# JeffOwOSun/ntm-tracker

Hardware: AMD Instinct MI355X
Metric: frames/sec (whole node) VGG16+NTM(128x20) seq_len=20 (higher is better)
Workload: dtype f32

## Files before the change

### ntm-tracker_amd/csrc/conv_bf16p.hip

```cpp
#include "conv_tiles.h"
#include "conv_stem.h"

#ifndef BF16P_ABL
#define BF16P_ABL 0
#endif

namespace {

typedef __bf16 pbf16x8 __attribute__((ext_vector_type(8)));
typedef __bf16 pbf16x4 __attribute__((ext_vector_type(4)));


struct Bf16pArgs {
    const __bf16* in; const __bf16* wq; const float* bias; void* out;
    int frames, H, W, Cin, Cout;
    int bxN, byN;
    int NQ, NS;
    int nCB;
    const float* stem_in = nullptr; const float* stem_w = nullptr; const float* stem_b = nullptr;
};

typedef int pv4i __attribute__((ext_vector_type(4)));
__device__ __forceinline__ void p_dma16(pv4i rs, unsigned lds_addr, int voff, int soff) {
    unsigned keep;
    asm volatile("s_mov_b32 %0, m0\n\ts_mov_b32 m0, %1\n\ts_nop 0\n\tbuffer_load_dwordx4 %2, %3, %4 offen lds\n\ts_mov_b32 m0, %0"
                 : "=&s"(keep) : "s"(lds_addr), "v"(voff), "s"(rs), "s"(soff) : "memory");
}
__device__ __forceinline__ pv4i p_rsrc(const void* base, unsigned bytes) {
    const unsigned long long p = (unsigned long long)base;
    return pv4i{(int)(unsigned)p, (int)(unsigned)(p >> 32), (int)bytes, 0x00020000};
}

__device__ __forceinline__ pbf16x8 p_as_bf16x8(const f32x4& v) {
    union { f32x4 f; pbf16x8 b; } u;
    u.f = v;
    return u.b;
}

typedef _Float16 ph16x8 __attribute__((ext_vector_type(8)));
typedef _Float16 ph16x4 __attribute__((ext_vector_type(4)));
typedef _Float16 ph16x2 __attribute__((ext_vector_type(2)));
__device__ __forceinline__ ph16x8 p_as_f16x8(const f32x4& v) {
    union { f32x4 f; ph16x8 h; } u;
    u.f = v;
    return u.h;
}
__device__ __forceinline__ void s3_split4(const f32x4& v, ph16x4& hi, ph16x4& lo) {
    const auto h01 = __builtin_amdgcn_cvt_pkrtz(v[0], v[1]), h23 = __builtin_amdgcn_cvt_pkrtz(v[2], v[3]);
    hi = ph16x4{(_Float16)h01[0], (_Float16)h01[1], (_Float16)h23[0], (_Float16)h23[1]};
#pragma unroll
    for (int e = 0; e < 4; ++e) lo[e] = (_Float16)(v[e] - (float)hi[e]);
}
constexpr float S3_MAX = 131008.f;

template <int PIECES>
__device__ __forceinline__ int p_sw(int idx) { return PIECES == 4 ? ((idx >> 2) & 3) : ((idx >> 3) & 1); }

template <int BN, int KC>
__global__ void bf16p_pack_kernel(const float* __restrict__ w, __bf16* __restrict__ wq, int Cin, int Cout) {
// ... 24 lines not shown
    for (int o = 32; o > 0; o >>= 1) m = fmaxf(m, __shfl_xor(m, o));
    if ((threadIdx.x & 63) == 0) atomicMax(tail + 1, __float_as_uint(m));
}
__global__ void split3_scale_kernel(unsigned* __restrict__ tail) {
    const float m = __uint_as_float(tail[1]);
    int e = 0;
    if (m > 0.f) frexpf(m, &e);
    int k = 14 - e;
    k = k > 100 ? 100 : (k < -100 ? -100 : k);
    reinterpret_cast<float*>(tail)[0] = ldexpf(1.f, -k);
    reinterpret_cast<float*>(tail)[2] = ldexpf(1.f, k);
}
template <int BN>
__global__ void split3_pack_kernel(const float* __restrict__ w, _Float16* __restrict__ wq, int Cin, int Cout) {
    const size_t total = (size_t)18 * Cin * Cout;
    const float wscale = reinterpret_cast<const float*>(wq + total)[2];
    const int NC = Cin / 16;
    for (size_t idx = (size_t)blockIdx.x * blockDim.x + threadIdx.x; idx < total; idx += (size_t)gridDim.x * blockDim.x) {
        const int e = idx & 7;
        size_t r = idx >> 3;
        const int slot = (int)(r & 3); r >>= 2;
        const int n = (int)(r % BN); r /= BN;
        const int tap = (int)(r % 9); r /= 9;
        const int chunk = (int)(r % NC);
        const int cb = (int)(r / NC);
        const int piece = slot ^ p_sw<4>(n);
        const int c = chunk * 16 + (piece & 1) * 8 + e;
        const float v = w[((size_t)tap * Cin + c) * Cout + (size_t)cb * BN + n] * wscale;
        const _Float16 hi = (_Float16)v;
        wq[idx] = (piece & 2) ? (_Float16)(v - (float)hi) : hi;
    }
}

template <int BN, int TW, int TH, int NSUB, int KC, bool POOL, bool OUTF32, int NW = 8, bool X3 = false, bool INF32 = false, bool STEM = false>
__global__ __launch_bounds__(64 * NW) __attribute__((amdgpu_waves_per_eu(2, 2))) void conv3x3_relu_bf16p_kernel(Bf16pArgs a) {
    static_assert(!INF32 || (X3 && NW == 4), "fp32 input: split form on four waves (the eight-wave form has no registers for the staging)");
    static_assert(!STEM || (X3 && NW == 4 && !INF32 && (TW & (TW - 1)) == 0 && TW % 2 == 0), "fused stem: split form on four waves, sub-blocks");
    constexpr int PNT = 2 * NW;
    constexpr bool ROWS = (TW & (TW - 1)) != 0;
    static_assert(!X3 || KC == 32, "split form: 16 real channels = one 32-channel chunk");
    static_assert(!ROWS || (!POOL && NSUB == 1 && (TW - 1 + 32 * PNT - 1) / TW + 1 <= TH - 1 && NW == 8), "runs of rows: no row pairs; TH = the patch's image rows");
    static_assert(NW == 8 || (NW == 4 && BN == 64), "four-wave workgroups take 64 columns");
    constexpr int PW = ROWS ? 32 : TW + 2, PH = TH + 2, SPX = PW * PH, NPX = NSUB * SPX;
    static_assert(!ROWS || TW + 2 <= 32, "runs of rows: the patch row pitch is 32");
    constexpr int PIXB = KC * 2, PIECES = KC / 8, PPP = 1024 / PIXB;
    constexpr int NPA = (NPX + PPP - 1) / PPP;
    constexpr int ABYTES = STEM ? NPX * PIXB : NPA * 1024;
    constexpr int STAPS = KC == 16 ? 9 : 3, SPC = 9 / STAPS;
    constexpr int SBYTES = STAPS * BN * PIXB, NPB = SBYTES / 1024;
    constexpr int NPAW = (NPA + NW - 1) / NW;
    constexpr int TM = BN == 128 ? 4 : 2;
    constexpr int TPS = (TW * TH) / 32;
    constexpr int K16 = KC / 16;
    static_assert(ROWS || NSUB * TW * TH == 32 * PNT, "512 (256) output pixels per workgroup");
    constexpr int TRB = POOL ? 0 : NW * TM * 32 * 144;
    constexpr int LDSB = (2 * ABYTES + 2 * SBYTES) > TRB ? (2 * ABYTES + 2 * SBYTES) : TRB;
    constexpr int FPW = TW + 4, FPN = STEM ? NSUB * (TH + 4) * FPW * 3 : 4;
    constexpr int STEMB = STEM ? (FPN + 4 * 27 * 16 + 64) * 4 : 0;
    static_assert(LDSB + STEMB + 1024 <= ((NW == 8 || (STEM && NSUB > 1)) ? 160 : 80) * 1024, "LDS");
    __shared__ __attribute__((aligned(16))) float s_fp[FPN];
    __shared__ __attribute__((aligned(16))) float s_w1[STEM ? 4 * 27 * 16 : 4];
    __shared__ __attribute__((aligned(16))) float s_b1[STEM ? 64 : 4];
    __shared__ __attribute__((aligned(1024))) unsigned char s_mem[LDSB];
    __shared__ int s_sbf[NSUB], s_sby[NSUB], s_sbx[NSUB];
    __shared__ __attribute__((aligned(16))) float s_bias[BN + 4];

    const int tid = threadIdx.x, lane = tid & 63;
    const int wave = __builtin_amdgcn_readfirstlane(tid >> 6);
    int cb, sp;
    conv_tile_wg(blockIdx.x, a.nCB, cb, sp);
    if (sp >= a.NS) return;
    const int H = a.H, W = a.W, Cin = a.Cin, Cout = a.Cout;
    const int rP0 = sp * (32 * PNT), rg0 = ROWS ? rP0 / TW : 0, rf0 = ROWS ? rg0 / H : 0, ry0 = ROWS ? rg0 - rf0 * H : 0;
    if (tid < BN) s_bias[tid] = a.bias[cb * BN + tid];
    if (X3 && tid == BN) s_bias[BN] = *reinterpret_cast<const float*>(a.wq + (size_t)9 * a.Cin * a.Cout);
    if constexpr (!ROWS) conv_tile_subblocks<NSUB>(s_sbf, s_sby, s_sbx, tid, sp, a.NQ, a.bxN, a.byN, TH, TW, 0, 0);
    if constexpr (STEM) {
        for (int e = tid; e < 4 * 27 * 16; e += 64 * NW) {
            const int k = (e >> 4) % 27;
            s_w1[e] = a.stem_w[((e / (27 * 16)) * 16 + (e & 15)) * 32 + k];
        }
        if (tid < 64) s_b1[tid] = a.stem_b[tid];
    }
    __syncthreads();
    if constexpr (STEM) {
        for (int e = tid; e < FPN; e += 64 * NW) {
            int q, fy, fx, c, y, x;
            stem_fp_elem(e, TW, TH, q, fy, fx, c);
            const bool in = stem_fp_src(fy, fx, s_sby[q], s_sbx[q], H, W, y, x) && s_sbf[q] >= 0;
            s_fp[e] = in ? a.stem_in[(((size_t)s_sbf[q] * H + y) * W + x) * 3 + c] : 0.f;
        }
        __syncthreads();
    }

    auto a_sw = [](int p) { return ROWS ? ((((p & 31) + 28 * (p >> 5)) >> 2) & 3) : p_sw<PIECES>(p); };
    const int f0 = ROWS ? rf0 : ((sp * NSUB) / a.bxN) / a.byN;
    const size_t in_left = (size_t)(a.frames - f0) * H * W * Cin * sizeof(__bf16);
    const unsigned in_bytes = (unsigned)(in_left < 0x7ffffff0ull ? in_left : 0x7ffffff0ull);
    const __bf16* pin = a.in + (size_t)f0 * H * W * Cin;
    unsigned aoff[NPAW];
#pragma unroll
    for (int i = 0; i < NPAW; ++i) {
        const int pa = wave + NW * i;
        const int lp = pa * PPP + lane / PIECES, slot = lane % PIECES;
        aoff[i] = 0x80000000u;
        if (pa < NPA && lp < NPX) {
            const int q = lp / SPX, rem = lp - q * SPX;
            const int py = rem / PW, px = rem - py * PW;
            int fq, y;
            const int x = (ROWS ? 0 : s_sbx[q]) - 1 + px;
            if constexpr (ROWS) {
                const int U = ry0 + py, df = U / (H + 1);
                fq = rf0 + df; y = U - df * (H + 1) - 1;
                if (fq >= a.frames) fq = -1;
            } else {
                fq = s_sbf[q]; y = s_sby[q] - 1 + py;
            }
            if (fq >= 0 && y >= 0 && y < H && x >= 0 && x < W)
                aoff[i] = (unsigned)(((((size_t)(fq - f0) * H + y) * W + x) * Cin + (slot ^ a_sw(lp)) * 8) * sizeof(__bf16));
        }
    }
    constexpr int NIT = INF32 ? (NPX * 4 + 64 * NW - 1) / (64 * NW) : 1;
    constexpr int NITS = (NIT + SPC - 1) / SPC;
    unsigned foff[NIT];
    int fdst[NIT];
    if constexpr (INF32) {
#pragma unroll
        for (int i = 0; i < NIT; ++i) {
            const int it = tid + 64 * NW * i, lp = it >> 2, qd = it & 3;
            foff[i] = 0x80000000u; fdst[i] = -1;
            if (lp < NPX) {
                fdst[i] = lp * PIXB + (((qd >> 1) ^ a_sw(lp)) << 4) + (qd & 1) * 8;
                const int q = lp / SPX, rem = lp - q * SPX;
                const int py = rem / PW, px = rem - py * PW;
                const int fq = s_sbf[q];
                const int y = s_sby[q] - 1 + py, x = s_sbx[q] - 1 + px;
                if (fq >= 0 && y >= 0 && y < H && x >= 0 && x < W)
                    foff[i] = (unsigned)(((((size_t)(fq - f0) * H + y) * W + x) * Cin) * sizeof(__bf16) + qd * 16);
            }
        }
    }
    auto f32_rsrc = [&](int chunk) {
        return __builtin_amdgcn_make_buffer_rsrc(const_cast<__bf16*>(pin + (size_t)chunk * KC), 0, (int)(in_bytes - (unsigned)chunk * PIXB), 0x00020000);
    };
    auto f32_put = [&](const f32x4& v, int dst) {
        ph16x4 h, l;
        f32x4 c;
#pragma unroll
        for (int e = 0; e < 4; ++e) c[e] = __builtin_amdgcn_fmed3f(v[e], -S3_MAX, S3_MAX);
        s3_split4(c, h, l);
        *reinterpret_cast<ph16x4*>(s_mem + dst) = h;
        *reinterpret_cast<ph16x4*>(s_mem + (dst ^ 32)) = l;
    };
    constexpr int STILES = (NPX + 15) / 16;
// ... 67 lines not shown
    auto dma_weights = [&](int stage, int buf) {
#pragma unroll
        for (int i = 0; i < (NPB + NW - 1) / NW; ++i) {
            const int pb = wave + NW * i;
            if (pb < NPB) p_dma16(wrs, lds0 + 2 * ABYTES + buf * SBYTES + pb * 1024, lane * 16, stage * SBYTES + pb * 1024);
        }
    };

    const int wm = BN == 128 ? (wave >> 1) : wave, wn = BN == 128 ? (wave & 1) : 0;
    const int mcol = lane & 31, kh = lane >> 5;
    int pix0[TM];
    int opix[TM];
    auto locate = [&](int t, int m, int& pc, int& op) {
        if constexpr (ROWS) {
            const int P = rP0 + t * 32 + m;
            const int g = P / TW, x = P - g * TW, f = g / H, y = g - f * H;
            const bool real = f < a.frames;
            pc = real ? ((f - rf0) * (H + 1) + y + 1 - ry0) * PW + x + 1 : PW + 1;
            op = real ? P : -1;
        } else {
            int q, y, x;
            if constexpr (TPS == 0) {
                q = 2 * t + (m >> 4); y = (m >> 2) & 3; x = m & 3;
            } else {
                constexpr int RPT = 32 / TW;
                const int tl = t % TPS, j = m / TW;
                q = t / TPS;
                y = 2 * ((tl >> 1) * RPT + j) + (tl & 1);
                x = m % TW;
                if constexpr (TW == 16) x = (x + 12 * j) & 15;
                if constexpr (TW == 8) x ^= ((0x9 >> j) & 1) << 2;
            }
            pc = q * SPX + (y + 1) * PW + (x + 1);
            const int fq = s_sbf[q];
            const int Y = s_sby[q] + y, X = s_sbx[q] + x;
            if constexpr (POOL) op = fq < 0 ? -1 : ((fq * (H >> 1) + (Y >> 1)) * (W >> 1) + (X >> 1));
            else op = fq < 0 ? -1 : ((fq * H + Y) * W + X);
        }
    };
#pragma unroll
    for (int tm = 0; tm < TM; ++tm) locate(wm * TM + tm, mcol, pix0[tm], opix[tm]);
    int xa[9][TM];
#pragma unroll
    for (int tap = 0; tap < 9; ++tap)
#pragma unroll
        for (int tm = 0; tm < TM; ++tm) {
            const int p = pix0[tm] + (tap / 3 - 1) * PW + (tap % 3 - 1);
            xa[tap][tm] = p * PIXB + ((kh ^ a_sw(p)) << 4);
        }
    f32x16 acc[TM][2];
#pragma unroll
    for (int tm = 0; tm < TM; ++tm)
#pragma unroll
        for (int nt = 0; nt < 2; ++nt)
#pragma unroll
            for (int r = 0; r < 16; ++r) acc[tm][nt][r] = 0.f;
    const int wa0 = 2 * ABYTES + (wn * 64 + mcol) * PIXB + ((kh ^ p_sw<PIECES>(mcol)) << 4);

    if constexpr (INF32) {
        const __amdgpu_buffer_rsrc_t rs = f32_rsrc(0);
        f32x4 v[NIT];
#pragma unroll
        for (int i = 0; i < NIT; ++i) v[i] = __builtin_bit_cast(f32x4, __builtin_amdgcn_raw_buffer_load_b128(rs, (int)foff[i], 0, 0));
#pragma unroll
        for (int i = 0; i < NIT; ++i)
            if (fdst[i] >= 0) f32_put(v[i], fdst[i]);
    } else if constexpr (!STEM) {
        dma_patch(0, 0, 0, NPAW);
    }
    dma_weights(0, 0);
    if constexpr (STEM) {
#pragma unroll
        for (int i = 0; i < SNIT; ++i) {
            stem_load(0, i, 0);
#pragma unroll
            for (int s = 0; s < 7; ++s) stem_mfma(0, s);
            stem_put(i, 0, 0);
        }
    }
    asm volatile("s_waitcnt vmcnt(0)" ::: "memory");
    __syncthreads();

    auto stage_body = [&](int chunk, auto part_c) {
        constexpr int part = decltype(part_c)::value;
        const int s = SPC * chunk + part;
        const int abuf = chunk & 1, bbuf = s & 1;
        constexpr int NDW = (NPB + NW - 1) / NW;
        constexpr int NDP = (INF32 || STEM) ? 0 : (NPAW + SPC - 1) / SPC;
        const bool more_w = !(BF16P_ABL & 1) && s + 1 < NSTG, more_p = !(BF16P_ABL & 1) && chunk + 1 < NC;
        auto dma_slot = [&](auto kc) {
            constexpr int k = decltype(kc)::value;
            if constexpr (k < NDW) { if (more_w) dma_weights1(s + 1, bbuf ^ 1, k); }
            else if constexpr (k < NDW + NDP && part * NDP + (k - NDW) < NPAW) {
                if (more_p) dma_patch1(chunk + 1, abuf ^ 1, ntk_ic<part * NDP + (k - NDW)>{});
            }
        };
        constexpr int SPER = (7 * SNITS + 8) / 9;
        auto stem_slot = [&](auto kc) {
            if constexpr (STEM) {
                constexpr int k = decltype(kc)::value;
                if (more_p) {
#pragma unroll
                    for (int u = k * SPER; u < (k + 1) * SPER && u < 7 * SNITS; ++u) {
                        if (part * SNITS + u / 7 >= SNIT) continue;
                        stem_mfma(u / 7, u % 7);
                        if (u % 7 == 6) stem_put(part * SNITS + u / 7, u / 7, abuf ^ 1);
                    }
                }
            }
        };
        if constexpr (STEM) {
            if (more_p) {
#pragma unroll
                for (int j = 0; j < SNITS; ++j)
                    if (part * SNITS + j < SNIT) stem_load(chunk + 1, part * SNITS + j, j);
            }
        }
        const int wa = wa0 + bbuf * SBYTES;
        f32x4 fst[NITS];
        if constexpr (INF32) {
            const __amdgpu_buffer_rsrc_t rs = f32_rsrc(more_p ? chunk + 1 : chunk);
#pragma unroll
            for (int j = 0; j < NITS; ++j)
                if (part * NITS + j < NIT) fst[j] = __builtin_bit_cast(f32x4, __builtin_amdgcn_raw_buffer_load_b128(rs, (int)foff[part * NITS + j], 0, 0));
        }
        if constexpr (X3) {
            f32x4 wh[2][2], wl[2], xh[TM], xl[TM];
// ... 30 lines not shown
                __builtin_amdgcn_sched_barrier(0);
                if constexpr (!(BF16P_ABL & 4)) ld_x(dc, I1{}, xl);
                __builtin_amdgcn_sched_barrier(0);
                mm(wl, xh);
                dma_slot(ntk_ic<3 * dxi + 1>{});
                stem_slot(ntk_ic<3 * dxi + 1>{});
                __builtin_amdgcn_sched_barrier(0);
                if constexpr (dxi + 1 < STAPS && !(BF16P_ABL & 4)) {
                    ld_w(ntk_ic<dxi + 1>{}, I0{}, wh[(dxi + 1) & 1]);
                    ld_x(ntk_ic<dxi + 1>{}, I0{}, xh);
                }
                __builtin_amdgcn_sched_barrier(0);
                mm(wh[dxi & 1], xl);
                dma_slot(ntk_ic<3 * dxi + 2>{});
                stem_slot(ntk_ic<3 * dxi + 2>{});
                __builtin_amdgcn_sched_barrier(0);
            };
            ld_w(I0{}, I0{}, wh[0]);
            ld_x(I0{}, I0{}, xh);
            if constexpr ((BF16P_ABL & 4) != 0) {
#pragma unroll
                for (int nt = 0; nt < 2; ++nt) { wh[1][nt] = wh[0][nt]; wl[nt] = wh[0][nt]; }
#pragma unroll
                for (int tm = 0; tm < TM; ++tm) xl[tm] = xh[tm];
            }
            ntk_static_for<0, STAPS>(tapstep);
            if constexpr (INF32) {
                if (more_p) {
#pragma unroll
                    for (int j = 0; j < NITS; ++j)
                        if (part * NITS + j < NIT && fdst[part * NITS + j] >= 0) f32_put(fst[j], (abuf ^ 1) * ABYTES + fdst[part * NITS + j]);
                }
            }
            if (!(BF16P_ABL & 2)) {
                asm volatile("s_waitcnt vmcnt(0)" ::: "memory");
                __syncthreads();
            }
            return;
        }
        constexpr int NSTEP = STAPS * K16;
        f32x4 wf[2][2], xf[2][TM];
        auto load_frags = [&](auto stc, f32x4 (&wfs)[2], f32x4 (&xfs)[TM]) {
            constexpr int st = decltype(stc)::value, dxi = st / K16, k16 = st % K16;
            constexpr int tap = part * STAPS + dxi;
#pragma unroll
            for (int nt = 0; nt < 2; ++nt)
                wfs[nt] = *reinterpret_cast<const f32x4*>(s_mem + ((wa ^ (k16 << 5)) + (dxi * BN + nt * 32) * PIXB));
#pragma unroll
            for (int tm = 0; tm < TM; ++tm) xfs[tm] = *reinterpret_cast<const f32x4*>(s_mem + (xa[tap][tm] ^ (k16 << 5)));
        };
        auto step = [&](auto stc) {
            constexpr int st = decltype(stc)::value;
            if constexpr (st + 1 < NSTEP && !(BF16P_ABL & 4)) load_frags(ntk_ic<st + 1>{}, wf[(st + 1) & 1], xf[(st + 1) & 1]);
            __builtin_amdgcn_sched_barrier(0);
            if constexpr ((BF16P_ABL & 8) != 0) return;
#pragma unroll
            for (int tm = 0; tm < TM; ++tm)
#pragma unroll
                for (int nt = 0; nt < 2; ++nt)
                    acc[tm][nt] = __builtin_amdgcn_mfma_f32_32x32x16_bf16(p_as_bf16x8(wf[(BF16P_ABL & 4) ? 0 : (st & 1)][nt]),
                                                                          p_as_bf16x8(xf[(BF16P_ABL & 4) ? 0 : (st & 1)][tm]), acc[tm][nt], 0, 0, 0);
            constexpr int PER = (NDW + NDP + NSTEP - 1) / NSTEP;
            dma_slot(ntk_ic<st * PER>{});
            if constexpr (PER > 1) dma_slot(ntk_ic<st * PER + 1>{});
            static_assert(PER <= 2, "DMAs per step");
            __builtin_amdgcn_sched_barrier(0);
        };
        if (!(BF16P_ABL & 4) || s == 0) load_frags(ntk_ic<0>{}, wf[0], xf[0]);
        ntk_static_for<0, NSTEP>(step);
        if (!(BF16P_ABL & 2)) {
            asm volatile("s_waitcnt vmcnt(0)" ::: "memory");
            __syncthreads();
        }
    };
    for (int chunk = 0; chunk < NC; ++chunk) {
        stage_body(chunk, ntk_ic<0>{});
        if constexpr (SPC > 1) {
            stage_body(chunk, ntk_ic<1>{});
            stage_body(chunk, ntk_ic<2>{});
        }
        const int flip = (chunk & 1) ? -ABYTES : ABYTES;
#pragma unroll
        for (int tap = 0; tap < 9; ++tap)
#pragma unroll
            for (int tm = 0; tm < TM; ++tm) xa[tap][tm] += flip;
    }

    if constexpr ((BF16P_ABL & 16) != 0) {
        float sacc = 0.f;
#pragma unroll
        for (int tm = 0; tm < TM; ++tm)
#pragma unroll
            for (int nt = 0; nt < 2; ++nt)
#pragma unroll
                for (int r = 0; r < 16; ++r) sacc += acc[tm][nt][r];
        if (sacc == 12345.f) reinterpret_cast<float*>(a.out)[tid] = sacc;
        return;
    }
    const int nbase = cb * BN + wn * 64 + 4 * kh;
    const float oscale = X3 ? s_bias[BN] : 1.f;
    if constexpr (POOL) {
#pragma unroll
        for (int nt = 0; nt < 2; ++nt)
#pragma unroll
            for (int g = 0; g < 4; ++g) {
                const int n = nbase + nt * 32 + 8 * g;
                const f32x4 bv = *reinterpret_cast<const f32x4*>(s_bias + n - cb * BN);
#pragma unroll
                for (int tm = 0; tm < TM; tm += 2) {
                    f32x4 v;
#pragma unroll
                    for (int e = 0; e < 4; ++e) {
                        const float m2 = fmaxf(acc[tm][nt][4 * g + e], acc[tm + 1][nt][4 * g + e]);
                        const float m4 = fmaxf(m2, ntk_dpp<0xB1>(m2));
                        if constexpr (X3 && !OUTF32) v[e] = __builtin_amdgcn_fmed3f(m4 * oscale + bv[e], 0.f, S3_MAX);
                        else v[e] = fmaxf((X3 ? m4 * oscale : m4) + bv[e], 0.f);
                    }
                    if (opix[tm] >= 0 && (mcol & 1) == 0) {
                        if constexpr (OUTF32) *reinterpret_cast<f32x4*>(reinterpret_cast<float*>(a.out) + (size_t)opix[tm] * Cout + n) = v;
                        else if constexpr (X3) {
                            ph16x4 oh, ol;
                            s3_split4(v, oh, ol);
                            _Float16* op = reinterpret_cast<_Float16*>(a.out) + (size_t)opix[tm] * (2 * Cout) + (n >> 4) * 32 + (n & 15);
                            *reinterpret_cast<ph16x4*>(op) = oh;
                            *reinterpret_cast<ph16x4*>(op + 16) = ol;
                        } else {
                            pbf16x4 o;
#pragma unroll
                            for (int e = 0; e < 4; ++e) o[e] = (__bf16)v[e];
                            *reinterpret_cast<pbf16x4*>(reinterpret_cast<__bf16*>(a.out) + (size_t)opix[tm] * Cout + n) = o;
                        }
                    }
                }
            }
    } else {
        constexpr int RB = 144;
        constexpr int WREG = TM * 32 * RB;
        static_assert(NW * WREG <= LDSB, "the transpose image fits");
        unsigned char* tr = s_mem + wave * WREG;
        constexpr bool WIDE = OUTF32 || X3;
        constexpr int NPASS = WIDE ? 2 : 1;
#pragma unroll
        for (int ps = 0; ps < NPASS; ++ps) {
#pragma unroll
            for (int nt = 0; nt < 2; ++nt) {
                if (WIDE && nt != ps) continue;
#pragma unroll
                for (int g = 0; g < 4; ++g) {
                    const f32x4 bv = *reinterpret_cast<const f32x4*>(s_bias + nbase - cb * BN + nt * 32 + 8 * g);
#pragma unroll
                    for (int tm = 0; tm < TM; ++tm) {
                        f32x4 v;
#pragma unroll
                        for (int e = 0; e < 4; ++e) {
                            if constexpr (X3 && !OUTF32) v[e] = __builtin_amdgcn_fmed3f(acc[tm][nt][4 * g + e] * oscale + bv[e], 0.f, S3_MAX);
                            else v[e] = fmaxf((X3 ? acc[tm][nt][4 * g + e] * oscale : acc[tm][nt][4 * g + e]) + bv[e], 0.f);
                        }
                        unsigned char* row = tr + (tm * 32 + mcol) * RB;
                        if constexpr (OUTF32) *reinterpret_cast<f32x4*>(row + (8 * g + 4 * kh) * 4) = v;
                        else if constexpr (X3) {
                            ph16x4 oh, ol;
                            s3_split4(v, oh, ol);
                            unsigned char* pr = row + (g >> 1) * 64 + ((g & 1) * 8 + 4 * kh) * 2;
                            *reinterpret_cast<ph16x4*>(pr) = oh;
                            *reinterpret_cast<ph16x4*>(pr + 32) = ol;
                        } else {
                            pbf16x4 o;
#pragma unroll
                            for (int e = 0; e < 4; ++e) o[e] = (__bf16)v[e];
                            *reinterpret_cast<pbf16x4*>(row + (nt * 32 + 8 * g + 4 * kh) * 2) = o;
                        }
                    }
                }
            }
#pragma unroll
            for (int j = 0; j < TM * 4; ++j) {
                const int tmr = j >> 2, mr = 8 * (j & 3) + (lane >> 3), piece = lane & 7;
                const f32x4 v = *reinterpret_cast<const f32x4*>(tr + (tmr * 32 + mr) * RB + piece * 16);
                const int opx = __builtin_amdgcn_ds_bpermute(mr << 2, opix[tmr]);
                if ((BF16P_ABL & 32) ? (opx >= 0 && v[0] == 12345.f) : (opx >= 0)) {
                    const size_t op = (size_t)opx * Cout + cb * BN + wn * 64;
                    if constexpr (OUTF32) *reinterpret_cast<f32x4*>(reinterpret_cast<float*>(a.out) + op + ps * 32 + piece * 4) = v;
                    else if constexpr (X3) *reinterpret_cast<f32x4*>(reinterpret_cast<__bf16*>(a.out) + 2 * (op + ps * 32) + piece * 8) = v;
                    else *reinterpret_cast<f32x4*>(reinterpret_cast<__bf16*>(a.out) + op + piece * 8) = v;
                }
            }
        }
    }
}

template <int BN, int KC, int NW, bool X3 = false, bool INF32 = false, bool STEM = false>
int bf16p_launch(const Bf16pArgs& a0, int H, int W, int pool, int out_f32, hipStream_t st) {
    Bf16pArgs a = a0;
    if constexpr (X3 && !INF32) {
        if (W == 28) {
            if (pool || NW != 8 || H < 20) return NTK_ERR_UNSUPPORTED;
            a.bxN = 1; a.byN = 1;
            const long long NQ = (long long)a.frames * H * W, NS = (NQ + 511) / 512;
            a.NQ = 0; a.NS = (int)NS; a.nCB = a.Cout / BN;
            const unsigned grid = (unsigned)conv_tile_grid(NS, a.nCB);
            if constexpr (NW == 8) {
                if (out_f32) conv3x3_relu_bf16p_kernel<BN, 28, 21, 1, 32, false, true, 8, true><<<grid, 512, 0, st>>>(a);
                else conv3x3_relu_bf16p_kernel<BN, 28, 21, 1, 32, false, false, 8, true><<<grid, 512, 0, st>>>(a);
            }
            return NTK_OK;
        }
    }
    int shape;
    if (NW == 8) shape = (W % 32 == 0 && H % 16 == 0) ? 0 : ((W % 16 == 0 && H % 16 == 0) ? 1 : ((W % 8 == 0 && H % 8 == 0) ? 2 : 3));
    else shape = (W % 32 == 0 && H % 8 == 0) ? 0 : ((W % 16 == 0 && H % 16 == 0) ? 1 : ((W % 8 == 0 && H % 8 == 0) ? 2 : 3));
    static const int TWs[4] = {32, 16, 8, 4}, THs8[4] = {16, 16, 8, 4}, THs4[4] = {8, 16, 8, 4}, NSUB8[4] = {1, 2, 8, 32}, NSUB4[4] = {1, 1, 4, 16};
    const int TWv = TWs[shape], THv = NW == 8 ? THs8[shape] : THs4[shape], NSUBv = NW == 8 ? NSUB8[shape] : NSUB4[shape];
    a.bxN = W / TWv;
    a.byN = H / THv;
    const long long NQ = (long long)a.frames * a.bxN * a.byN;
    const long long NS = (NQ + NSUBv - 1) / NSUBv;
    a.NQ = (int)NQ; a.NS = (int)NS; a.nCB = a.Cout / BN;
    const unsigned grid = (unsigned)conv_tile_grid(NS, a.nCB);
#define BF16P_GO(TW_, TH_, NSUB_)                                                                                             \
    do {                                                                                                                      \
        if (pool) {                                                                                                           \
            if (out_f32) conv3x3_relu_bf16p_kernel<BN, TW_, TH_, NSUB_, KC, true, true, NW, X3, INF32, STEM><<<grid, 64 * NW, 0, st>>>(a);     \
            else conv3x3_relu_bf16p_kernel<BN, TW_, TH_, NSUB_, KC, true, false, NW, X3, INF32, STEM><<<grid, 64 * NW, 0, st>>>(a);            \
        } else {                                                                                                              \
            if (out_f32) conv3x3_relu_bf16p_kernel<BN, TW_, TH_, NSUB_, KC, false, true, NW, X3, INF32, STEM><<<grid, 64 * NW, 0, st>>>(a);    \
            else conv3x3_relu_bf16p_kernel<BN, TW_, TH_, NSUB_, KC, false, false, NW, X3, INF32, STEM><<<grid, 64 * NW, 0, st>>>(a);           \
        }                                                                                                                     \
    } while (0)
    if constexpr (KC == 32 && NW == 8) {
        if (shape == 0) BF16P_GO(32, 16, 1);
        else if (shape == 1) BF16P_GO(16, 16, 2);
        else if (shape == 2) BF16P_GO(8, 8, 8);
        else return NTK_ERR_UNSUPPORTED;
    } else if constexpr (KC == 32) {
        if (shape == 0) BF16P_GO(32, 8, 1);
        else if (shape == 1) BF16P_GO(16, 16, 1);
        else if (shape == 2) BF16P_GO(8, 8, 4);
        else return NTK_ERR_UNSUPPORTED;
    } else {
        if (shape == 3 && !pool && NW == 8) {
            if (out_f32) conv3x3_relu_bf16p_kernel<BN, 4, 4, 32, KC, false, true><<<grid, 512, 0, st>>>(a);
            else conv3x3_relu_bf16p_kernel<BN, 4, 4, 32, KC, false, false><<<grid, 512, 0, st>>>(a);
        } else return NTK_ERR_UNSUPPORTED;
    }
#undef BF16P_GO
    return NTK_OK;
}

}

static int bf16p_form(int H, int W, int cin, int cout, int pool, int* bn, int* kc, int* nw) {
    if (H <= 0 || W <= 0 || cin <= 0 || cout <= 0 || (H % 4) || (W % 4) || cin % 32 || cout % 64) return 0;
    const bool rect = (W % 8 == 0 && H % 8 == 0);
    if (!rect && pool) return 0;
    *nw = (rect && cin <= 64 && cout == 64) ? 4 : 8;
    *bn = (*nw == 8 && cout % 128 == 0) ? 128 : 64;
    *kc = rect ? 32 : 16;
    return conv_tile_ncb_ok(cout / *bn);
}

extern "C" size_t ntk_vgg_bf16p_packed_elems(int cin, int cout) { return (size_t)9 * cin * cout; }

extern "C" int ntk_vgg_pack_weights_bf16p(const float* w_hwio, void* w_packed_bf16, int cin, int cout, int H, int W, void* stream) {
    NTK_REQUIRE(w_hwio && w_packed_bf16, NTK_ERR_BAD_PTR, "ntk_vgg_pack_weights_bf16p: null pointer");
    int bn = 0, kc = 0, nw = 0;
    NTK_REQUIRE(bf16p_form(H, W, cin, cout, 0, &bn, &kc, &nw), NTK_ERR_UNSUPPORTED,
                "ntk_vgg_pack_weights_bf16p: cin=%d (multiple of 32) cout=%d (multiple of 64) H=%d W=%d (multiples of 4)", cin, cout, H, W);
    __bf16* wq = reinterpret_cast<__bf16*>(w_packed_bf16);
    hipStream_t st = (hipStream_t)stream;
    if (bn == 128 && kc == 32) bf16p_pack_kernel<128, 32><<<1024, 256, 0, st>>>(w_hwio, wq, cin, cout);
    else if (bn == 64 && kc == 32) bf16p_pack_kernel<64, 32><<<1024, 256, 0, st>>>(w_hwio, wq, cin, cout);
    else if (bn == 128) bf16p_pack_kernel<128, 16><<<1024, 256, 0, st>>>(w_hwio, wq, cin, cout);
    else bf16p_pack_kernel<64, 16><<<1024, 256, 0, st>>>(w_hwio, wq, cin, cout);
    NTK_CHECK_LAUNCH("ntk_vgg_pack_weights_bf16p");
    return NTK_OK;
// ... 121 lines not shown
```

Baseline: 13830.

## Make bf16 conv3x3 kernel persistent with atomic tile claiming and cross-tile prefetch

```diff
diff --git a/ntm-tracker_amd/csrc/conv_bf16p.hip b/ntm-tracker_amd/csrc/conv_bf16p.hip
--- a/ntm-tracker_amd/csrc/conv_bf16p.hip
+++ b/ntm-tracker_amd/csrc/conv_bf16p.hip
@@ -1,3 +1,5 @@
+#include <stdlib.h>
+#include <string.h>
 #include "conv_tiles.h"
 #include "conv_stem.h"
 
@@ -18,6 +20,8 @@
     int NQ, NS;
     int nCB;
     const float* stem_in = nullptr; const float* stem_w = nullptr; const float* stem_b = nullptr;
+    int* ctr = nullptr;
+    int NT = 0;
 };
 
 typedef int pv4i __attribute__((ext_vector_type(4)));
@@ -25,6 +29,9 @@
     unsigned keep;
     asm volatile("s_mov_b32 %0, m0\n\ts_mov_b32 m0, %1\n\ts_nop 0\n\tbuffer_load_dwordx4 %2, %3, %4 offen lds\n\ts_mov_b32 m0, %0"
                  : "=&s"(keep) : "s"(lds_addr), "v"(voff), "s"(rs), "s"(soff) : "memory");
+}
+__device__ __forceinline__ void p_claim_issue(int* ctr, int& r) {
+    asm volatile("global_atomic_add %0, %1, %2, off sc0" : "=&v"(r) : "v"(ctr), "v"(1) : "memory");
 }
 __device__ __forceinline__ pv4i p_rsrc(const void* base, unsigned bytes) {
     const unsigned long long p = (unsigned long long)base;
@@ -115,8 +122,10 @@
     }
 }
 
-template <int BN, int TW, int TH, int NSUB, int KC, bool POOL, bool OUTF32, int NW = 8, bool X3 = false, bool INF32 = false, bool STEM = false>
+template <int BN, int TW, int TH, int NSUB, int KC, bool POOL, bool OUTF32, int NW = 8, bool X3 = false, bool INF32 = false, bool STEM = false,
+          bool LOOP = false>
 __global__ __launch_bounds__(64 * NW) __attribute__((amdgpu_waves_per_eu(2, 2))) void conv3x3_relu_bf16p_kernel(Bf16pArgs a) {
+    static_assert(!LOOP || (!INF32 && !STEM && KC == 32), "tile loop: the DMA-staged forms with three stages per chunk");
     static_assert(!INF32 || (X3 && NW == 4), "fp32 input: split form on four waves (the eight-wave form has no registers for the staging)");
     static_assert(!STEM || (X3 && NW == 4 && !INF32 && (TW & (TW - 1)) == 0 && TW % 2 == 0), "fused stem: split form on four waves, sub-blocks");
     constexpr int PNT = 2 * NW;
@@ -145,7 +154,9 @@
     __shared__ __attribute__((aligned(16))) float s_w1[STEM ? 4 * 27 * 16 : 4];
     __shared__ __attribute__((aligned(16))) float s_b1[STEM ? 64 : 4];
     __shared__ __attribute__((aligned(1024))) unsigned char s_mem[LDSB];
-    __shared__ int s_sbf[NSUB], s_sby[NSUB], s_sbx[NSUB];
+    constexpr int NTB = LOOP ? 2 : 1;
+    __shared__ int s_sbf[NTB * NSUB], s_sby[NTB * NSUB], s_sbx[NTB * NSUB];
+    __shared__ int s_claim;
     __shared__ __attribute__((aligned(16))) float s_bias[BN + 4];
 
     const int tid = threadIdx.x, lane = tid & 63;
@@ -153,8 +164,22 @@
     int cb, sp;
     conv_tile_wg(blockIdx.x, a.nCB, cb, sp);
     if (sp >= a.NS) return;
+    if constexpr (LOOP) {
+        if (tid == 0) s_claim = atomicAdd(a.ctr + cb, 1);
+        __syncthreads();
+        sp = __builtin_amdgcn_readfirstlane(s_claim);
+        if (sp >= a.NT) return;
+    }
+    const int NT = LOOP ? a.NT : a.NS;
     const int H = a.H, W = a.W, Cin = a.Cin, Cout = a.Cout;
-    const int rP0 = sp * (32 * PNT), rg0 = ROWS ? rP0 / TW : 0, rf0 = ROWS ? rg0 / H : 0, ry0 = ROWS ? rg0 - rf0 * H : 0;
+    int rP0, rf0, ry0, rf0d = 0, ry0d = 0;
+    auto rows_origin = [&](int spx, int& P0, int& f0x, int& y0x) {
+        P0 = spx * (32 * PNT);
+        const int g0 = ROWS ? P0 / TW : 0;
+        f0x = ROWS ? g0 / H : 0; y0x = ROWS ? g0 - f0x * H : 0;
+    };
+    rows_origin(sp, rP0, rf0, ry0);
+    int tbo = 0;
     if (tid < BN) s_bias[tid] = a.bias[cb * BN + tid];
     if (X3 && tid == BN) s_bias[BN] = *reinterpret_cast<const float*>(a.wq + (size_t)9 * a.Cin * a.Cout);
     if constexpr (!ROWS) conv_tile_subblocks<NSUB>(s_sbf, s_sby, s_sbx, tid, sp, a.NQ, a.bxN, a.byN, TH, TW, 0, 0);
@@ -177,32 +202,41 @@
     }
 
     auto a_sw = [](int p) { return ROWS ? ((((p & 31) + 28 * (p >> 5)) >> 2) & 3) : p_sw<PIECES>(p); };
-    const int f0 = ROWS ? rf0 : ((sp * NSUB) / a.bxN) / a.byN;
-    const size_t in_left = (size_t)(a.frames - f0) * H * W * Cin * sizeof(__bf16);
-    const unsigned in_bytes = (unsigned)(in_left < 0x7ffffff0ull ? in_left : 0x7ffffff0ull);
-    const __bf16* pin = a.in + (size_t)f0 * H * W * Cin;
+    int f0;
+    unsigned in_bytes;
+    const __bf16* pin;
     unsigned aoff[NPAW];
-#pragma unroll
-    for (int i = 0; i < NPAW; ++i) {
-        const int pa = wave + NW * i;
-        const int lp = pa * PPP + lane / PIECES, slot = lane % PIECES;
-        aoff[i] = 0x80000000u;
-        if (pa < NPA && lp < NPX) {
-            const int q = lp / SPX, rem = lp - q * SPX;
-            const int py = rem / PW, px = rem - py * PW;
-            int fq, y;
-            const int x = (ROWS ? 0 : s_sbx[q]) - 1 + px;
-            if constexpr (ROWS) {
-                const int U = ry0 + py, df = U / (H + 1);
-                fq = rf0 + df; y = U - df * (H + 1) - 1;
-                if (fq >= a.frames) fq = -1;
-            } else {
-                fq = s_sbf[q]; y = s_sby[q] - 1 + py;
-            }
-            if (fq >= 0 && y >= 0 && y < H && x >= 0 && x < W)
-                aoff[i] = (unsigned)(((((size_t)(fq - f0) * H + y) * W + x) * Cin + (slot ^ a_sw(lp)) * 8) * sizeof(__bf16));
-        }
-    }
+    auto patch_src = [&](int spx, int tb) {
+        int lane_o = lane, wave_o = wave;
+        if constexpr (LOOP) asm volatile("" : "+v"(lane_o), "+s"(wave_o));
+        if constexpr (ROWS) { int P0; rows_origin(spx, P0, rf0d, ry0d); }
+        f0 = ROWS ? rf0d : ((spx * NSUB) / a.bxN) / a.byN;
+        const size_t in_left = (size_t)(a.frames - f0) * H * W * Cin * sizeof(__bf16);
+        in_bytes = (unsigned)(in_left < 0x7ffffff0ull ? in_left : 0x7ffffff0ull);
+        pin = a.in + (size_t)f0 * H * W * Cin;
+#pragma unroll
+        for (int i = 0; i < NPAW; ++i) {
+            const int pa = wave_o + NW * i;
+            const int lp = pa * PPP + lane_o / PIECES, slot = lane_o % PIECES;
+            aoff[i] = 0x80000000u;
+            if (pa < NPA && lp < NPX) {
+                const int q = lp / SPX, rem = lp - q * SPX;
+                const int py = rem / PW, px = rem - py * PW;
+                int fq, y;
+                const int x = (ROWS ? 0 : s_sbx[tb + q]) - 1 + px;
+                if constexpr (ROWS) {
+                    const int U = ry0d + py, df = U / (H + 1);
+                    fq = rf0d + df; y = U - df * (H + 1) - 1;
+                    if (fq >= a.frames) fq = -1;
+                } else {
+                    fq = s_sbf[tb + q]; y = s_sby[tb + q] - 1 + py;
+                }
+                if (fq >= 0 && y >= 0 && y < H && x >= 0 && x < W)
+                    aoff[i] = (unsigned)(((((size_t)(fq - f0) * H + y) * W + x) * Cin + (slot ^ a_sw(lp)) * 8) * sizeof(__bf16));
+            }
+        }
+    };
+    patch_src(sp, 0);
     constexpr int NIT = INF32 ? (NPX * 4 + 64 * NW - 1) / (64 * NW) : 1;
     constexpr int NITS = (NIT + SPC - 1) / SPC;
     unsigned foff[NIT];
@@ -336,8 +370,8 @@
                 if constexpr (TW == 8) x ^= ((0x9 >> j) & 1) << 2;
             }
             pc = q * SPX + (y + 1) * PW + (x + 1);
-            const int fq = s_sbf[q];
-            const int Y = s_sby[q] + y, X = s_sbx[q] + x;
+            const int fq = s_sbf[tbo + q];
+            const int Y = s_sby[tbo + q] + y, X = s_sbx[tbo + q] + x;
             if constexpr (POOL) op = fq < 0 ? -1 : ((fq * (H >> 1) + (Y >> 1)) * (W >> 1) + (X >> 1));
             else op = fq < 0 ? -1 : ((fq * H + Y) * W + X);
         }
@@ -345,20 +379,27 @@
 #pragma unroll
     for (int tm = 0; tm < TM; ++tm) locate(wm * TM + tm, mcol, pix0[tm], opix[tm]);
     int xa[9][TM];
-#pragma unroll
-    for (int tap = 0; tap < 9; ++tap)
-#pragma unroll
-        for (int tm = 0; tm < TM; ++tm) {
-            const int p = pix0[tm] + (tap / 3 - 1) * PW + (tap % 3 - 1);
-            xa[tap][tm] = p * PIXB + ((kh ^ a_sw(p)) << 4);
-        }
+    auto frag_offsets = [&](int boff) {
+#pragma unroll
+        for (int tap = 0; tap < 9; ++tap)
+#pragma unroll
+            for (int tm = 0; tm < TM; ++tm) {
+                const int p = pix0[tm] + (tap / 3 - 1) * PW + (tap % 3 - 1);
+                xa[tap][tm] = p * PIXB + ((kh ^ a_sw(p)) << 4) + boff;
+            }
+    };
+    frag_offsets(0);
     f32x16 acc[TM][2];
-#pragma unroll
-    for (int tm = 0; tm < TM; ++tm)
-#pragma unroll
-        for (int nt = 0; nt < 2; ++nt)
-#pragma unroll
-            for (int r = 0; r < 16; ++r) acc[tm][nt][r] = 0.f;
+    auto acc_zero = [&]() {
+#pragma unroll
+        for (int tm = 0; tm < TM; ++tm)
+#pragma unroll
+            for (int nt = 0; nt < 2; ++nt)
+#pragma unroll
+                for (int r = 0; r < 16; ++r) acc[tm][nt][r] = 0.f;
+    };
+    acc_zero();
+    int par = 0, nsp = NT, nxt = 0;
     const int wa0 = 2 * ABYTES + (wn * 64 + mcol) * PIXB + ((kh ^ p_sw<PIECES>(mcol)) << 4);
 
     if constexpr (INF32) {
@@ -388,15 +429,28 @@
     auto stage_body = [&](int chunk, auto part_c) {
         constexpr int part = decltype(part_c)::value;
         const int s = SPC * chunk + part;
-        const int abuf = chunk & 1, bbuf = s & 1;
+        const int abuf = (chunk + par) & 1, bbuf = (s + par) & 1;
+        if constexpr (LOOP && part == 0) {
+            if (chunk == 0 && tid == 0) p_claim_issue(a.ctr + cb, nxt);
+        }
+        if constexpr (LOOP && part == 1) {
+            if (chunk == 0) {
+                nsp = __builtin_amdgcn_readfirstlane(s_claim);
+                if constexpr (!ROWS) {
+                    if (nsp < NT) conv_tile_subblocks<NSUB>(s_sbf + (tbo ^ NSUB), s_sby + (tbo ^ NSUB), s_sbx + (tbo ^ NSUB), tid, nsp, a.NQ, a.bxN, a.byN, TH, TW, 0, 0);
+                }
+            }
+        }
+        const bool has_next = LOOP && nsp < NT;
         constexpr int NDW = (NPB + NW - 1) / NW;
         constexpr int NDP = (INF32 || STEM) ? 0 : (NPAW + SPC - 1) / SPC;
-        const bool more_w = !(BF16P_ABL & 1) && s + 1 < NSTG, more_p = !(BF16P_ABL & 1) && chunk + 1 < NC;
+        const bool more_w = !(BF16P_ABL & 1) && (s + 1 < NSTG || has_next), more_p = !(BF16P_ABL & 1) && (chunk + 1 < NC || has_next);
+        const int next_s = (LOOP && s + 1 >= NSTG) ? 0 : s + 1, next_c = (LOOP && chunk + 1 >= NC) ? 0 : chunk + 1;
         auto dma_slot = [&](auto kc) {
             constexpr int k = decltype(kc)::value;
-            if constexpr (k < NDW) { if (more_w) dma_weights1(s + 1, bbuf ^ 1, k); }
+            if constexpr (k < NDW) { if (more_w) dma_weights1(next_s, bbuf ^ 1, k); }
             else if constexpr (k < NDW + NDP && part * NDP + (k - NDW) < NPAW) {
-                if (more_p) dma_patch1(chunk + 1, abuf ^ 1, ntk_ic<part * NDP + (k - NDW)>{});
+                if (more_p) dma_patch1(next_c, abuf ^ 1, ntk_ic<part * NDP + (k - NDW)>{});
             }
         };
         constexpr int SPER = (7 * SNITS + 8) / 9;
@@ -493,6 +547,12 @@
                         if (part * NITS + j < NIT && fdst[part * NITS + j] >= 0) f32_put(fst[j], (abuf ^ 1) * ABYTES + fdst[part * NITS + j]);
                 }
             }
+            if constexpr (LOOP && part == 0) {
+                if (chunk == 0 && tid == 0) {
+                    asm volatile("s_waitcnt vmcnt(0)" : "+v"(nxt) : : "memory");
+                    s_claim = nxt;
+                }
+            }
             if (!(BF16P_ABL & 2)) {
                 asm volatile("s_waitcnt vmcnt(0)" ::: "memory");
                 __syncthreads();
@@ -529,125 +589,232 @@
         };
         if (!(BF16P_ABL & 4) || s == 0) load_frags(ntk_ic<0>{}, wf[0], xf[0]);
         ntk_static_for<0, NSTEP>(step);
+        if constexpr (LOOP && part == 0) {
+            if (chunk == 0 && tid == 0) {
+                asm volatile("s_waitcnt vmcnt(0)" : "+v"(nxt) : : "memory");
+                s_claim = nxt;
+            }
+        }
         if (!(BF16P_ABL & 2)) {
             asm volatile("s_waitcnt vmcnt(0)" ::: "memory");
             __syncthreads();
         }
     };
-    for (int chunk = 0; chunk < NC; ++chunk) {
-        stage_body(chunk, ntk_ic<0>{});
-        if constexpr (SPC > 1) {
-            stage_body(chunk, ntk_ic<1>{});
-            stage_body(chunk, ntk_ic<2>{});
-        }
-        const int flip = (chunk & 1) ? -ABYTES : ABYTES;
-#pragma unroll
-        for (int tap = 0; tap < 9; ++tap)
-#pragma unroll
-            for (int tm = 0; tm < TM; ++tm) xa[tap][tm] += flip;
-    }
-
-    if constexpr ((BF16P_ABL & 16) != 0) {
-        float sacc = 0.f;
-#pragma unroll
-        for (int tm = 0; tm < TM; ++tm)
+    auto tile_chunks = [&]() {
+        for (int chunk = 0; chunk < NC; ++chunk) {
+            if constexpr (LOOP) {
+                if (chunk + 1 == NC && nsp < NT) patch_src(nsp, tbo ^ NSUB);
+            }
+            stage_body(chunk, ntk_ic<0>{});
+            if constexpr (SPC > 1) {
+                stage_body(chunk, ntk_ic<1>{});
+                stage_body(chunk, ntk_ic<2>{});
+            }
+            const int flip = ((chunk + par) & 1) ? -ABYTES : ABYTES;
+#pragma unroll
+            for (int tap = 0; tap < 9; ++tap)
+#pragma unroll
+                for (int tm = 0; tm < TM; ++tm) xa[tap][tm] += flip;
+        }
+    };
+
+    auto epilogue = [&]() {
+        if constexpr ((BF16P_ABL & 16) != 0) {
+            float sacc = 0.f;
+#pragma unroll
+            for (int tm = 0; tm < TM; ++tm)
+#pragma unroll
+                for (int nt = 0; nt < 2; ++nt)
+#pragma unroll
+                    for (int r = 0; r < 16; ++r) sacc += acc[tm][nt][r];
+            if (sacc == 12345.f) reinterpret_cast<float*>(a.out)[tid] = sacc;
+            return;
+        }
+        int lane_e = lane, wave_e = wave;
+        if constexpr (LOOP) asm volatile("" : "+v"(lane_e), "+s"(wave_e));
+        const int mcol_e = lane_e & 31, kh_e = lane_e >> 5, wn_e = BN == 128 ? (wave_e & 1) : 0;
+        const int nbase = cb * BN + wn_e * 64 + 4 * kh_e;
+        const float oscale = X3 ? s_bias[BN] : 1.f;
+        if constexpr (POOL) {
 #pragma unroll
             for (int nt = 0; nt < 2; ++nt)
 #pragma unroll
-                for (int r = 0; r < 16; ++r) sacc += acc[tm][nt][r];
-        if (sacc == 12345.f) reinterpret_cast<float*>(a.out)[tid] = sacc;
-        return;
-    }
-    const int nbase = cb * BN + wn * 64 + 4 * kh;
-    const float oscale = X3 ? s_bias[BN] : 1.f;
-    if constexpr (POOL) {
-#pragma unroll
-        for (int nt = 0; nt < 2; ++nt)
-#pragma unroll
-            for (int g = 0; g < 4; ++g) {
-                const int n = nbase + nt * 32 + 8 * g;
-                const f32x4 bv = *reinterpret_cast<const f32x4*>(s_bias + n - cb * BN);
-#pragma unroll
-                for (int tm = 0; tm < TM; tm += 2) {
-                    f32x4 v;
-#pragma unroll
-                    for (int e = 0; e < 4; ++e) {
-                        const float m2 = fmaxf(acc[tm][nt][4 * g + e], acc[tm + 1][nt][4 * g + e]);
-                        const float m4 = fmaxf(m2, ntk_dpp<0xB1>(m2));
-                        if constexpr (X3 && !OUTF32) v[e] = __builtin_amdgcn_fmed3f(m4 * oscale + bv[e], 0.f, S3_MAX);
-                        else v[e] = fmaxf((X3 ? m4 * oscale : m4) + bv[e], 0.f);
-                    }
-                    if (opix[tm] >= 0 && (mcol & 1) == 0) {
-                        if constexpr (OUTF32) *reinterpret_cast<f32x4*>(reinterpret_cast<float*>(a.out) + (size_t)opix[tm] * Cout + n) = v;
-                        else if constexpr (X3) {
-                            ph16x4 oh, ol;
-                            s3_split4(v, oh, ol);
-                            _Float16* op = reinterpret_cast<_Float16*>(a.out) + (size_t)opix[tm] * (2 * Cout) + (n >> 4) * 32 + (n & 15);
-                            *reinterpret_cast<ph16x4*>(op) = oh;
-                            *reinterpret_cast<ph16x4*>(op + 16) = ol;
-                        } else {
-                            pbf16x4 o;
-#pragma unroll
-                            for (int e = 0; e < 4; ++e) o[e] = (__bf16)v[e];
-                            *reinterpret_cast<pbf16x4*>(reinterpret_cast<__bf16*>(a.out) + (size_t)opix[tm] * Cout + n) = o;
+                for (int g = 0; g < 4; ++g) {
+                    const int n = nbase + nt * 32 + 8 * g;
+                    const f32x4 bv = *reinterpret_cast<const f32x4*>(s_bias + n - cb * BN);
+#pragma unroll
+                    for (int tm = 0; tm < TM; tm += 2) {
+                        f32x4 v;
+#pragma unroll
+                        for (int e = 0; e < 4; ++e) {
+                            const float m2 = fmaxf(acc[tm][nt][4 * g + e], acc[tm + 1][nt][4 * g + e]);
+                            const float m4 = fmaxf(m2, ntk_dpp<0xB1>(m2));
+                            if constexpr (X3 && !OUTF32) v[e] = __builtin_amdgcn_fmed3f(m4 * oscale + bv[e], 0.f, S3_MAX);
+                            else v[e] = fmaxf((X3 ? m4 * oscale : m4) + bv[e], 0.f);
+                        }
+                        if (opix[tm] >= 0 && (mcol_e & 1) == 0) {
+                            if constexpr (OUTF32) *reinterpret_cast<f32x4*>(reinterpret_cast<float*>(a.out) + (size_t)opix[tm] * Cout + n) = v;
+                            else if constexpr (X3) {
+                                ph16x4 oh, ol;
+                                s3_split4(v, oh, ol);
+                                _Float16* op = reinterpret_cast<_Float16*>(a.out) + (size_t)opix[tm] * (2 * Cout) + (n >> 4) * 32 + (n & 15);
+                                *reinterpret_cast<ph16x4*>(op) = oh;
+                                *reinterpret_cast<ph16x4*>(op + 16) = ol;
+                            } else {
+                                pbf16x4 o;
+#pragma unroll
+                                for (int e = 0; e < 4; ++e) o[e] = (__bf16)v[e];
+                                *reinterpret_cast<pbf16x4*>(reinterpret_cast<__bf16*>(a.out) + (size_t)opix[tm] * Cout + n) = o;
+                            }
                         }
                     }
                 }
-            }
-    } else {
-        constexpr int RB = 144;
-        constexpr int WREG = TM * 32 * RB;
-        static_assert(NW * WREG <= LDSB, "the transpose image fits");
-        unsigned char* tr = s_mem + wave * WREG;
-        constexpr bool WIDE = OUTF32 || X3;
-        constexpr int NPASS = WIDE ? 2 : 1;
-#pragma unroll
-        for (int ps = 0; ps < NPASS; ++ps) {
-#pragma unroll
-            for (int nt = 0; nt < 2; ++nt) {
-                if (WIDE && nt != ps) continue;
-#pragma unroll
-                for (int g = 0; g < 4; ++g) {
-                    const f32x4 bv = *reinterpret_cast<const f32x4*>(s_bias + nbase - cb * BN + nt * 32 + 8 * g);
-#pragma unroll
-                    for (int tm = 0; tm < TM; ++tm) {
-                        f32x4 v;
-#pragma unroll
-                        for (int e = 0; e < 4; ++e) {
-                            if constexpr (X3 && !OUTF32) v[e] = __builtin_amdgcn_fmed3f(acc[tm][nt][4 * g + e] * oscale + bv[e], 0.f, S3_MAX);
-                            else v[e] = fmaxf((X3 ? acc[tm][nt][4 * g + e] * oscale : acc[tm][nt][4 * g + e]) + bv[e], 0.f);
-                        }
-                        unsigned char* row = tr + (tm * 32 + mcol) * RB;
-                        if constexpr (OUTF32) *reinterpret_cast<f32x4*>(row + (8 * g + 4 * kh) * 4) = v;
-                        else if constexpr (X3) {
-                            ph16x4 oh, ol;
-                            s3_split4(v, oh, ol);
-                            unsigned char* pr = row + (g >> 1) * 64 + ((g & 1) * 8 + 4 * kh) * 2;
-                            *reinterpret_cast<ph16x4*>(pr) = oh;
-                            *reinterpret_cast<ph16x4*>(pr + 32) = ol;
-                        } else {
-                            pbf16x4 o;
-#pragma unroll
-                            for (int e = 0; e < 4; ++e) o[e] = (__bf16)v[e];
-                            *reinterpret_cast<pbf16x4*>(row + (nt * 32 + 8 * g + 4 * kh) * 2) = o;
+        } else {
+            constexpr int RB = 144;
+            constexpr int TG = LOOP ? 1 : TM;
+            constexpr int WREG = TG * 32 * RB;
+            static_assert(NW * WREG <= (LOOP ? ABYTES : LDSB), "the transpose image fits");
+            unsigned char* tr = s_mem + (LOOP ? ((NC - 1 + par) & 1) * ABYTES : 0) + wave_e * WREG;
+            constexpr bool WIDE = OUTF32 || X3;
+            constexpr int NPASS = WIDE ? 2 : 1;
+#pragma unroll
+            for (int ps = 0; ps < NPASS; ++ps)
+#pragma unroll
+            for (int t0 = 0; t0 < TM; t0 += TG) {
+#pragma unroll
+                for (int nt = 0; nt < 2; ++nt) {
+                    if (WIDE && nt != ps) continue;
+#pragma unroll
+                    for (int g = 0; g < 4; ++g) {
+                        const f32x4 bv = *reinterpret_cast<const f32x4*>(s_bias + nbase - cb * BN + nt * 32 + 8 * g);
+#pragma unroll
+                        for (int tm = t0; tm < t0 + TG; ++tm) {
+                            f32x4 v;
+#pragma unroll
+                            for (int e = 0; e < 4; ++e) {
+                                if constexpr (X3 && !OUTF32) v[e] = __builtin_amdgcn_fmed3f(acc[tm][nt][4 * g + e] * oscale + bv[e], 0.f, S3_MAX);
+                                else v[e] = fmaxf((X3 ? acc[tm][nt][4 * g + e] * oscale : acc[tm][nt][4 * g + e]) + bv[e], 0.f);
+                            }
+                            unsigned char* row = tr + ((tm - t0) * 32 + mcol_e) * RB;
+                            if constexpr (OUTF32) *reinterpret_cast<f32x4*>(row + (8 * g + 4 * kh_e) * 4) = v;
+                            else if constexpr (X3) {
+                                ph16x4 oh, ol;
+                                s3_split4(v, oh, ol);
+                                unsigned char* pr = row + (g >> 1) * 64 + ((g & 1) * 8 + 4 * kh_e) * 2;
+                                *reinterpret_cast<ph16x4*>(pr) = oh;
+                                *reinterpret_cast<ph16x4*>(pr + 32) = ol;
+                            } else {
+                                pbf16x4 o;
+#pragma unroll
+                                for (int e = 0; e < 4; ++e) o[e] = (__bf16)v[e];
+                                *reinterpret_cast<pbf16x4*>(row + (nt * 32 + 8 * g + 4 * kh_e) * 2) = o;
+                            }
                         }
                     }
                 }
-            }
-#pragma unroll
-            for (int j = 0; j < TM * 4; ++j) {
-                const int tmr = j >> 2, mr = 8 * (j & 3) + (lane >> 3), piece = lane & 7;
-                const f32x4 v = *reinterpret_cast<const f32x4*>(tr + (tmr * 32 + mr) * RB + piece * 16);
-                const int opx = __builtin_amdgcn_ds_bpermute(mr << 2, opix[tmr]);
-                if ((BF16P_ABL & 32) ? (opx >= 0 && v[0] == 12345.f) : (opx >= 0)) {
-                    const size_t op = (size_t)opx * Cout + cb * BN + wn * 64;
-                    if constexpr (OUTF32) *reinterpret_cast<f32x4*>(reinterpret_cast<float*>(a.out) + op + ps * 32 + piece * 4) = v;
-                    else if constexpr (X3) *reinterpret_cast<f32x4*>(reinterpret_cast<__bf16*>(a.out) + 2 * (op + ps * 32) + piece * 8) = v;
-                    else *reinterpret_cast<f32x4*>(reinterpret_cast<__bf16*>(a.out) + op + piece * 8) = v;
+#pragma unroll
+                for (int j = 0; j < TG * 4; ++j) {
+                    const int tmr = t0 + (j >> 2), mr = 8 * (j & 3) + (lane_e >> 3), piece = lane_e & 7;
+                    const f32x4 v = *reinterpret_cast<const f32x4*>(tr + ((j >> 2) * 32 + mr) * RB + piece * 16);
+                    const int opx = __builtin_amdgcn_ds_bpermute(mr << 2, opix[tmr]);
+                    if ((BF16P_ABL & 32) ? (opx >= 0 && v[0] == 12345.f) : (opx >= 0)) {
+                        const size_t op = (size_t)opx * Cout + cb * BN + wn_e * 64;
+                        if constexpr (OUTF32) *reinterpret_cast<f32x4*>(reinterpret_cast<float*>(a.out) + op + ps * 32 + piece * 4) = v;
+                        else if constexpr (X3) *reinterpret_cast<f32x4*>(reinterpret_cast<__bf16*>(a.out) + 2 * (op + ps * 32) + piece * 8) = v;
+                        else *reinterpret_cast<f32x4*>(reinterpret_cast<__bf16*>(a.out) + op + piece * 8) = v;
+                    }
                 }
             }
         }
-    }
+    };
+
+    for (;;) {
+        tile_chunks();
+        epilogue();
+        if constexpr (!LOOP) return;
+        if (nsp >= NT) return;
+        sp = nsp; tbo ^= NSUB; par = (par + NC) & 1;
+        rows_origin(sp, rP0, rf0, ry0);
+        int mcol_o = mcol, wm_o = wm;
+        asm volatile("" : "+v"(mcol_o), "+s"(wm_o));
+#pragma unroll
+        for (int tm = 0; tm < TM; ++tm) locate(wm_o * TM + tm, mcol_o, pix0[tm], opix[tm]);
+        if constexpr (ROWS) frag_offsets(par * ABYTES);
+        acc_zero();
+        if constexpr (!POOL) asm volatile("s_waitcnt lgkmcnt(0)\n\ts_barrier" ::: "memory");
+    }
+}
+
+constexpr int CLAIM_RING = 4096, CLAIM_CB = 16;
+static int bf16p_claim_slot(hipStream_t st, int** ctr) {
+    static int* ring[64];
+    static unsigned next[64];
+    int dev = 0;
+    hipError_t e = hipGetDevice(&dev);
+    if (e == hipSuccess && (dev < 0 || dev >= 64)) e = hipErrorInvalidDevice;
+    int* r = nullptr;
+    if (e == hipSuccess) {
+        r = __atomic_load_n(&ring[dev], __ATOMIC_ACQUIRE);
+        if (!r) {
+            int* fresh = nullptr;
+            e = hipMalloc(reinterpret_cast<void**>(&fresh), (size_t)CLAIM_RING * CLAIM_CB * sizeof(int));
+            if (e == hipSuccess) {
+                int* seen = nullptr;
+                if (__atomic_compare_exchange_n(&ring[dev], &seen, fresh, false, __ATOMIC_ACQ_REL, __ATOMIC_ACQUIRE)) r = fresh;
+                else { (void)hipFree(fresh); r = seen; }
+            }
+        }
+    }
+    if (e == hipSuccess) {
+        r += (size_t)(__atomic_fetch_add(&next[dev], 1u, __ATOMIC_RELAXED) % CLAIM_RING) * CLAIM_CB;
+        e = hipMemsetAsync(r, 0, CLAIM_CB * sizeof(int), st);
+    }
+    if (e != hipSuccess) {
+        (void)hipGetLastError();
+        ntk_set_error("conv3x3 tile loop: claim counters: %s", hipGetErrorString(e));
+        return NTK_ERR_HIP;
+    }
+    *ctr = r;
+    return NTK_OK;
+}
+static int bf16p_tile_loop(int nw, int nCB, long long tiles, int* wgs) {
+    const char* form = getenv("NTK_TRUNK_TILES");
+    if (form && *form && strcmp(form, "loop") != 0) {
+        NTK_REQUIRE(strcmp(form, "single") == 0, NTK_ERR_UNSUPPORTED, "NTK_TRUNK_TILES must be 'loop' or 'single'");
+        return 0;
+    }
+    if (nCB > CLAIM_CB) return 0;
+    const int cus = ntk_device_cu_count();
+    NTK_REQUIRE(cus > 0, NTK_ERR_HIP, "conv3x3 tile loop: no device");
+    long long n = (long long)cus * (nw == 4 ? 2 : 1) / nCB;
+    if (n < 1) n = 1;
+    const char* cap = getenv("NTK_TRUNK_TILE_WGS");
+    if (cap && *cap) {
+        const int c = atoi(cap);
+        NTK_REQUIRE(c > 0, NTK_ERR_UNSUPPORTED, "NTK_TRUNK_TILE_WGS must be a positive number");
+        if (c < n) n = c;
+    }
+    *wgs = (int)(tiles < n ? tiles : n);
+    return 1;
+}
+
+template <int BN, int TW, int TH, int NSUB, int KC, bool POOL, bool OUTF32, int NW, bool X3, bool INF32, bool STEM>
+int bf16p_go(Bf16pArgs a, hipStream_t st) {
+    if constexpr (KC == 32 && !INF32 && !STEM) {
+        int wgs = 0;
+        const int loop = a.Cin / KC >= 2 ? bf16p_tile_loop(NW, a.nCB, a.NS, &wgs) : 0;
+        if (loop < 0) return loop;
+        if (loop) {
+            const int rc = bf16p_claim_slot(st, &a.ctr);
+            if (rc != NTK_OK) return rc;
+            a.NT = a.NS; a.NS = wgs;
+            conv3x3_relu_bf16p_kernel<BN, TW, TH, NSUB, KC, POOL, OUTF32, NW, X3, INF32, STEM, true>
+                <<<(unsigned)conv_tile_grid(a.NS, a.nCB), 64 * NW, 0, st>>>(a);
+            return NTK_OK;
+        }
+    }
+    conv3x3_relu_bf16p_kernel<BN, TW, TH, NSUB, KC, POOL, OUTF32, NW, X3, INF32, STEM><<<(unsigned)conv_tile_grid(a.NS, a.nCB), 64 * NW, 0, st>>>(a);
+    return NTK_OK;
 }
 
 template <int BN, int KC, int NW, bool X3 = false, bool INF32 = false, bool STEM = false>
@@ -659,10 +826,9 @@
             a.bxN = 1; a.byN = 1;
             const long long NQ = (long long)a.frames * H * W, NS = (NQ + 511) / 512;
             a.NQ = 0; a.NS = (int)NS; a.nCB = a.Cout / BN;
-            const unsigned grid = (unsigned)conv_tile_grid(NS, a.nCB);
             if constexpr (NW == 8) {
-                if (out_f32) conv3x3_relu_bf16p_kernel<BN, 28, 21, 1, 32, false, true, 8, true><<<grid, 512, 0, st>>>(a);
-                else conv3x3_relu_bf16p_kernel<BN, 28, 21, 1, 32, false, false, 8, true><<<grid, 512, 0, st>>>(a);
+                return out_f32 ? bf16p_go<BN, 28, 21, 1, 32, false, true, 8, true, false, false>(a, st)
+                               : bf16p_go<BN, 28, 21, 1, 32, false, false, 8, true, false, false>(a, st);
             }
             return NTK_OK;
         }
@@ -677,17 +843,11 @@
     const long long NQ = (long long)a.frames * a.bxN * a.byN;
     const long long NS = (NQ + NSUBv - 1) / NSUBv;
     a.NQ = (int)NQ; a.NS = (int)NS; a.nCB = a.Cout / BN;
-    const unsigned grid = (unsigned)conv_tile_grid(NS, a.nCB);
 #define BF16P_GO(TW_, TH_, NSUB_)                                                                                             \
-    do {                                                                                                                      \
-        if (pool) {                                                                                                           \
-            if (out_f32) conv3x3_relu_bf16p_kernel<BN, TW_, TH_, NSUB_, KC, true, true, NW, X3, INF32, STEM><<<grid, 64 * NW, 0, st>>>(a);     \
-            else conv3x3_relu_bf16p_kernel<BN, TW_, TH_, NSUB_, KC, true, false, NW, X3, INF32, STEM><<<grid, 64 * NW, 0, st>>>(a);            \
-        } else {                                                                                                              \
-            if (out_f32) conv3x3_relu_bf16p_kernel<BN, TW_, TH_, NSUB_, KC, false, true, NW, X3, INF32, STEM><<<grid, 64 * NW, 0, st>>>(a);    \
-            else conv3x3_relu_bf16p_kernel<BN, TW_, TH_, NSUB_, KC, false, false, NW, X3, INF32, STEM><<<grid, 64 * NW, 0, st>>>(a);           \
-        }                                                                                                                     \
-    } while (0)
+    return pool ? (out_f32 ? bf16p_go<BN, TW_, TH_, NSUB_, KC, true, true, NW, X3, INF32, STEM>(a, st)                        \
+                           : bf16p_go<BN, TW_, TH_, NSUB_, KC, true, false, NW, X3, INF32, STEM>(a, st))                      \
+                : (out_f32 ? bf16p_go<BN, TW_, TH_, NSUB_, KC, false, true, NW, X3, INF32, STEM>(a, st)                       \
+                           : bf16p_go<BN, TW_, TH_, NSUB_, KC, false, false, NW, X3, INF32, STEM>(a, st))
     if constexpr (KC == 32 && NW == 8) {
         if (shape == 0) BF16P_GO(32, 16, 1);
         else if (shape == 1) BF16P_GO(16, 16, 2);
@@ -700,8 +860,8 @@
         else return NTK_ERR_UNSUPPORTED;
     } else {
         if (shape == 3 && !pool && NW == 8) {
-            if (out_f32) conv3x3_relu_bf16p_kernel<BN, 4, 4, 32, KC, false, true><<<grid, 512, 0, st>>>(a);
-            else conv3x3_relu_bf16p_kernel<BN, 4, 4, 32, KC, false, false><<<grid, 512, 0, st>>>(a);
+            return out_f32 ? bf16p_go<BN, 4, 4, 32, KC, false, true, 8, false, false, false>(a, st)
+                           : bf16p_go<BN, 4, 4, 32, KC, false, false, 8, false, false, false>(a, st);
         } else return NTK_ERR_UNSUPPORTED;
     }
 #undef BF16P_GO
```

Measured after the change: 12990. 0.94x the previous value.
